# tpoisonooo/how-to-optimize-gemm

Measured on NVIDIA H100. Metric: SGEMM GFLOP/s (square N=4096 point of the 256..4096 sweep), higher is better.
Workload: dtype f16x2(scaled split-f32)

## Files before the change

how-to-optimize-gemm_b200/csrc/capi.cu:

```cuda
#include "../../include/b200gemm.h"

#include <cuda.h>
#include <cuda_runtime.h>
#include <stdio.h>
#include <stdlib.h>
#include <string.h>

#include <atomic>
#include <mutex>
#include <vector>

#include "gemm_ffma.cuh"
#include "gemm_generic.cuh"
#include "gemm_mxf4.cuh"
#include "gemm_tc.cuh"

using namespace b200;

namespace {

std::atomic<unsigned long long> g_launches{0};
int g_split_tail = 1;

struct KernelTimer {
// ... 58 lines not shown
  unsigned flag_slot = 0;
  struct FlagUser {
    cudaStream_t st = nullptr;
    cudaEvent_t ev = nullptr;
    bool used = false;
  } flag_user[kFlagSlots];
  std::mutex ws_mu;
  Scratch ws;
  cudaEvent_t ws_event = nullptr;
  cudaStream_t ws_stream = nullptr;
  bool ws_busy = false;
  struct MaxBuf {
    unsigned slot = 0;
    float* buf = nullptr;
    size_t cap = 0;
    int dirty[2] = {0, 0};
  } cmax, amax;
  cudaStream_t aux = nullptr;
  cudaEvent_t aux_fork = nullptr, aux_join = nullptr;
  std::mutex host_mu;
  Scratch scr[4];
  HostPipe pipe;
  std::vector<const void*> attr_done;
};
constexpr int kMaxDevices = 64;
DevCtx g_ctx[kMaxDevices];
std::mutex g_mu;

typedef CUresult (*EncodeTiledFn)(CUtensorMap*, CUtensorMapDataType, cuuint32_t, void*,
                                  const cuuint64_t*, const cuuint64_t*, const cuuint32_t*,
                                  const cuuint32_t*, CUtensorMapInterleave, CUtensorMapSwizzle,
                                  CUtensorMapL2promotion, CUtensorMapFloatOOBfill);
EncodeTiledFn g_encode = nullptr;

thread_local DevCtx* t_ctx = nullptr;
thread_local int t_bound_dev = -1;

int ensure_device() {
  int dev = -1;
  if (cudaGetDevice(&dev) != cudaSuccess || dev < 0 || dev >= kMaxDevices) { cudaGetLastError(); t_ctx = nullptr; return B200_ERR_NO_DEVICE; }
  if (t_bound_dev != dev) {
    if (cudaSetDevice(dev) != cudaSuccess) { cudaGetLastError(); t_ctx = nullptr; return B200_ERR_NO_DEVICE; }
    t_bound_dev = dev;
  }
  DevCtx* c = &g_ctx[dev];
  t_ctx = c;
// ... 25 lines not shown
  }
  for (auto& u : c->flag_user)
    if (!u.ev && cudaEventCreateWithFlags(&u.ev, cudaEventDisableTiming) != cudaSuccess) {
      cudaGetLastError(); u.ev = nullptr; c->ok = -1; return B200_ERR_NO_DEVICE;
    }
  c->dev = dev;
  c->sms = prop.multiProcessorCount;
  c->ok = 1;
  return 0;
}

template <typename Kern>
int ensure_smem_attr(Kern kern, int bytes) {
  const void* key = reinterpret_cast<const void*>(kern);
  {
    std::lock_guard<std::mutex> lk(g_mu);
    for (const void* k : t_ctx->attr_done) if (k == key) return 0;
  }
  cudaError_t e = cudaFuncSetAttribute(kern, cudaFuncAttributeMaxDynamicSharedMemorySize, bytes);
  if (e != cudaSuccess) { cudaGetLastError(); return (int)e; }
  std::lock_guard<std::mutex> lk(g_mu);
  t_ctx->attr_done.push_back(key);
  return 0;
}

struct MapKey {
  const void* ptr; int dtype; unsigned long long d0, d1, ld_bytes; unsigned b0, b1; int swz; int dev;
  unsigned long long d2, d2_bytes;
  bool operator==(const MapKey& o) const {
    return ptr == o.ptr && dtype == o.dtype && d0 == o.d0 && d1 == o.d1 && ld_bytes == o.ld_bytes &&
           b0 == o.b0 && b1 == o.b1 && swz == o.swz && dev == o.dev && d2 == o.d2 && d2_bytes == o.d2_bytes;
  }
};
struct MapEntry { MapKey key; CUtensorMap map; };
std::vector<MapEntry> g_maps;
size_t g_map_next = 0;
constexpr size_t kMapCache = 64;

int get_map(CUtensorMap* out, const void* ptr, CUtensorMapDataType dt, int elem_bytes,
            unsigned long long inner, unsigned long long rows, unsigned long long ld_bytes,
            unsigned box_inner, unsigned box_rows, int swizzle ,
            unsigned long long entries = 0, unsigned long long entry_bytes = 0) {
  MapKey key{ptr, (int)dt, inner, rows, ld_bytes, box_inner, box_rows, swizzle, t_ctx->dev, entries, entry_bytes};
  std::lock_guard<std::mutex> lk(g_mu);
  for (auto& e : g_maps)
    if (e.key == key) { *out = e.map; return 0; }
// ... 100 lines not shown
  if (cs == cudaStreamCaptureStatusNone) {
    if (u->used && (u->st != st || st == cudaStreamPerThread) && (e = cudaStreamWaitEvent(st, u->ev, 0)) != cudaSuccess) {
      cudaGetLastError();
      return (int)e;
    }
    *user = u;
  }
  if ((e = cudaMemsetAsync(*flags, 0, 1024 * sizeof(int), st)) != cudaSuccess) { cudaGetLastError(); return (int)e; }
  return 0;
}
void release_flag_slot(DevCtx::FlagUser* u, cudaStream_t st) {
  if (!u) return;
  if (cudaEventRecord(u->ev, st) != cudaSuccess) { cudaGetLastError(); return; }
  u->st = st;
  u->used = true;
}

int g_force_bn = 0;
int g_group_rows = 0;
constexpr int kStreamCDefault = 0;
int g_stream_c = -1;
int g_ffma_fat = -1;
int g_ffma_halves = 1;

struct Stack {
  int count;
  long long sa, sb, sc;
  const int32_t* offs;
};
long long grouped_tile_rows(int total_m, int groups) { return (total_m + 127LL) / 128 + groups; }

template <int KIND, int BN, int STAGES, typename OutT, class Prod = ProdSingle, int A_ROW_BYTES = 128, int AL = LAYOUT_K,
          int BL = KindTraits<KIND>::B_LAYOUT, bool EPI = false, int STACK = STACK_NONE, class ScaleT = TcScale>
int launch_tc(int m, int n, int k, const void* A, long long lda, int a_rows_total, int a_plane_rows,
              const void* B, long long ldb, int b_rows_total, int b_plane_rows, void* C, int ldc,
              const char* name, const Call& c, int chunk_k = 0, const float* row_max = nullptr,
              const float* col_max = nullptr, const Stack* stk = nullptr, const ScaleT* scl = nullptr) {
  using Cfg = TcConfig<KIND, BN, STAGES, Prod, A_ROW_BYTES, AL, BL>;
  using T = KindTraits<KIND>;
  constexpr bool FP8 = KIND == KIND_E4M3 || KIND == KIND_E4M3E5M2 || KIND == KIND_E5M2E4M3;
  constexpr bool BLK = std::is_same<ScaleT, TcBlockScale>::value || std::is_same<ScaleT, TcStackBlockScale>::value ||
                      std::is_same<ScaleT, TcBlockScaleQ8>::value;
  constexpr int smem = Cfg::SMEM_BYTES + (BLK ? STAGES * kBlkScaleStageBytes : 0);
  constexpr CUtensorMapDataType dt = KIND == KIND_F16 ? CU_TENSOR_MAP_DATA_TYPE_BFLOAT16
                                   : KIND == KIND_FP16 ? CU_TENSOR_MAP_DATA_TYPE_FLOAT16
                                   : KIND == KIND_TF32 ? CU_TENSOR_MAP_DATA_TYPE_FLOAT32
                                                       : CU_TENSOR_MAP_DATA_TYPE_UINT8;
  CUtensorMap tmA, tmB;
  constexpr int kswz = A_ROW_BYTES == 128 ? 1 : 3;
  unsigned long long ea = 0, eab = 0, eb = 0, ebb = 0;
  if constexpr (STACK != STACK_NONE) {
    const unsigned long long abytes = (unsigned long long)lda * T::ELEM, bbytes = (unsigned long long)ldb * T::ELEM;
    ea = stk->sa ? stk->count : 1; eab = stk->sa ? (unsigned long long)stk->sa * T::ELEM : a_rows_total * abytes;
    eb = stk->sb ? stk->count : 1; ebb = stk->sb ? (unsigned long long)stk->sb * T::ELEM : b_rows_total * bbytes;
  }
  int rc;
  if constexpr (Cfg::A_MN)
    rc = get_map(&tmA, A, dt, T::ELEM, m, a_rows_total, (unsigned long long)lda * T::ELEM, Cfg::MN_BOX_COLS, Cfg::BK, 1, ea,
                 eab);
  else
    rc = get_map(&tmA, A, dt, T::ELEM, k, a_rows_total, (unsigned long long)lda * T::ELEM, Cfg::BK, Cfg::BM, kswz, ea, eab);
  if (rc) return rc;
  if constexpr (!Cfg::B_MN)
// ... 5 lines not shown
  if (rc) return rc;
  TcParams p;
  p.C = C; p.ldc = ldc; p.M = m; p.N = n; p.K = k;
  p.tiles_m = STACK == STACK_GROUP ? (int)grouped_tile_rows(m, stk->count) : (m + Cfg::TILE_M - 1) / Cfg::TILE_M;
  p.tiles_n = (n + BN - 1) / BN;
  p.group_m = (g_group_rows > 0 ? g_group_rows : 2048) / Cfg::TILE_M;
  if (p.group_m < 1) p.group_m = 1;
  constexpr int OB = OutBytes<OutT>::V;
  p.vec_ok = aligned16(C) && ((long long)ldc * OB) % 16 == 0;
  if constexpr (STACK != STACK_NONE) p.vec_ok = p.vec_ok && stk->sc % (16 / OB) == 0;
  p.a_plane_rows = a_plane_rows; p.b_plane_rows = b_plane_rows;
  p.chunk_kb = chunk_k > 0 ? (chunk_k + Cfg::BK - 1) / Cfg::BK : (k + Cfg::BK - 1) / Cfg::BK;
  if (p.chunk_kb < 1) p.chunk_kb = 1;
  p.dbg_b_lbo = g_dbg_b_lbo; p.dbg_b_sbo = g_dbg_b_sbo;
  p.row_max = row_max; p.col_max = col_max;
  p.accumulate = c.acc;
  p.axpby = c.axpby; p.alpha = c.alpha; p.beta = c.beta;
  p.act = c.act;
  if constexpr (EPI) p.bias = c.bias;
  p.stream_c = g_stream_c < 0 ? (g_stream_c = (getenv("B200GEMM_STREAM_C") ? atoi(getenv("B200GEMM_STREAM_C")) : kStreamCDefault)) : g_stream_c;
  auto kern = [] {
    if constexpr (FP8) return gemm_tc_fp8_kernel<KIND, BN, STAGES, OutT, Prod, BLK, STACK>;
    else if constexpr (STACK != STACK_NONE) return gemm_tc_stacked_kernel<KIND, BN, STAGES, OutT, AL, BL, STACK>;
    else return gemm_tc_kernel<KIND, BN, STAGES, OutT, Prod, A_ROW_BYTES, AL, BL, EPI>;
  }();
  if (int arc = ensure_smem_attr(kern, smem)) return arc;
  TcStack ts{1, 0, 0, 0, nullptr};
  if constexpr (STACK != STACK_NONE) ts = TcStack{stk->count, stk->sa ? 1 : 0, stk->sb ? 1 : 0, stk->sc, stk->offs};
  [[maybe_unused]] ScaleT fp8_scale{};
  if constexpr (FP8) {
    fp8_scale = *scl;
    if constexpr (STACK != STACK_NONE) fp8_scale.st = ts;
  }
  int tiles = p.tiles_m * p.tiles_n * (STACK == STACK_GROUP ? 1 : ts.count);
  const int units_max = t_ctx->sms - c.sm_reserve > 2 ? t_ctx->sms - c.sm_reserve : t_ctx->sms;
  const int num_kb = (k + Cfg::BK - 1) / Cfg::BK;
  const int rem = tiles % units_max;
  int split = 1;
  if (!EPI && !FP8 && STACK != STACK_GROUP && STACK != STACK_KGROUP && g_split_tail && OB == 4 && rem > 0) {
    split = units_max / rem;
    if (split > 4) split = 4;
    if (split > num_kb / 8) split = num_kb / 8;
    if (split < 1) split = 1;
    if (rem * Cfg::EPI_WARPS > 1024) split = 1;
  }
  p.split = split;
  p.full_tiles = split > 1 ? tiles - rem : tiles;
  p.flags = t_ctx->flags;
  std::unique_lock<std::mutex> flag_lk;
  DevCtx::FlagUser* flag_user = nullptr;
  if (split > 1) {
    flag_lk = std::unique_lock<std::mutex>(t_ctx->flag_mu);
    if (int rc = take_flag_slot(c.st, &p.flags, &flag_user)) return rc;
  }
  const int items = p.full_tiles + (tiles - p.full_tiles) * split;
  const int units = items < units_max ? items : units_max;
  t_last_schedule = Schedule{tiles, split, p.full_tiles, units};
  g_ktimer.begin(c.st);
  {
    cudaError_t e;
    if constexpr (FP8) e = launch_pdl(kern, dim3(units), dim3(Cfg::THREADS), smem, c.st, 1, tmA, tmB, p, fp8_scale);
    else if constexpr (STACK != STACK_NONE) e = launch_pdl(kern, dim3(units), dim3(Cfg::THREADS), smem, c.st, 1, tmA, tmB, p, ts);
    else e = launch_pdl(kern, dim3(units), dim3(Cfg::THREADS), smem, c.st, 1, tmA, tmB, p);
    release_flag_slot(flag_user, c.st);
    if (e != cudaSuccess) { cudaGetLastError(); return (int)e; }
  }
  g_ktimer.end(c.st);
  g_launches++;
  t_last_kernel = name;
  return last_launch_status();
}

int pick_bn(int m, int n, bool allow256, bool allow192 = true, int batch = 1) {
  if (g_force_bn == 128 || (g_force_bn == 192 && allow192) || (g_force_bn == 256 && allow256)) return g_force_bn;
  const int cands[3] = {256, 192, 128};
  const double eff[3] = {1.00, 0.97, 0.80};
  int best = 128;
  double best_cost = 1e300;
  const int tm = (m + 127) / 128;
  for (int i = 0; i < 3; i++) {
    if (cands[i] == 256 && !allow256) continue;
    if (cands[i] == 192 && !allow192) continue;
    const long long tiles = (long long)tm * ((n + cands[i] - 1) / cands[i]) * batch;
    const long long waves = (tiles + t_ctx->sms - 1) / t_ctx->sms;
    const double cost = (double)waves * (cands[i] / eff[i] + 8.0);
    if (cost < best_cost) { best_cost = cost; best = cands[i]; }
// ... 214 lines not shown
  if (gy < 1) gy = 1;
  launch_pdl(split_planes_kernel<NP>, dim3(gx, gy, jobs), dim3(256), 0, st, 1, ja, jb);
  g_launches += 1;
  return last_launch_status();
}

struct PlaneGeom {
  int rows, cols, plane_rows;
  long long pitch;
  size_t bytes(int np) const { return (size_t)np * plane_rows * pitch * 2; }
};
inline PlaneGeom plane_geom(bool k_along_rows, int rows, int cols) {
  return PlaneGeom{rows, cols, k_along_rows ? b_plane_rows(rows) : rows, plane_pitch(cols)};
}
inline PlaneGeom geom_a(int op_a, int m, int k) { return op_a ? plane_geom(true, k, m) : plane_geom(false, m, k); }
inline PlaneGeom geom_b(int op_b, int k, int n) { return op_b ? plane_geom(false, n, k) : plane_geom(true, k, n); }

size_t split_ws_bytes(int np, int op_a, int op_b, int m, int n, int k, bool prepB = false) {
  const size_t a = round1024(geom_a(op_a, m, k).bytes(np));
  return prepB ? a : a + geom_b(op_b, k, n).bytes(np);
}

KernelNames kNamesBf16x3 = TC_NAMES("tc_bf16x3"), kNamesBf16x2 = TC_NAMES("tc_bf16x2"), kNamesF16x2 = TC_NAMES("tc_f16x2");

template <int NP>
int gemm_f32_split(int op_a, int op_b, int m, int n, int k, const float* A, int lda, const float* B, int ldb, float* C,
                   int ldc, const uint16_t* prepB, const Call& c) {
  const PlaneGeom ga = geom_a(op_a, m, k), gb = geom_b(op_b, k, n);
  WsLease ws(split_ws_bytes(NP, op_a, op_b, m, n, k, prepB != nullptr), c.st);
  if (ws.rc) return ws.rc;
  uint16_t* pA = reinterpret_cast<uint16_t*>(ws.base());
  const uint16_t* pB = prepB ? prepB : reinterpret_cast<uint16_t*>(ws.base() + round1024(ga.bytes(NP)));
  const SplitJob ja{A, lda, ga.rows, ga.cols, pA, ga.pitch, ga.plane_rows},
                 jb{B, ldb, gb.rows, gb.cols, const_cast<uint16_t*>(pB), gb.pitch, gb.plane_rows};
  if (int rc = launch_split<NP>(ja, jb, prepB ? 1 : 2, c.st)) return rc;
  using Prod = typename std::conditional<NP == 3, ProdX3, ProdX2>::type;
  return with_layout(op_a, op_b, [&](auto L) {
    using Lay = decltype(L);
    return launch_tc<KIND_F16, 128, NP == 3 ? 4 : 6, float, Prod, 64, Lay::AL, Lay::BL>(
        m, n, k, pA, ga.pitch, NP * ga.plane_rows, ga.plane_rows, pB, gb.pitch, NP * gb.plane_rows, gb.plane_rows, C, ldc,
        (NP == 3 ? kNamesBf16x3 : kNamesBf16x2)[Lay::idx][2], c, g_split_chunk_k[NP == 3 ? 0 : 1]);
  });
}

struct F16Operand {
  const uint16_t* planes;
  long long pitch;
  int plane_rows;
  const float* maxv;
};

int launch_f16_split_rows(const float* A, long long lda, int rows, int cols, float* rmax, uint16_t* planes,
                          long long pitch, int plane_rows, cudaStream_t st) {
  int blocks = (plane_rows + 7) / 8;
  const int cap = t_ctx->sms * 16;
  if (blocks > cap) blocks = cap;
  if (blocks < 1) blocks = 1;
  if (cols <= 1024) launch_pdl(split_f16_rows_kernel<4>, dim3(blocks), dim3(256), 0, st, 1, A, (long long)lda, rows, cols, rmax, planes, pitch, plane_rows);
  else if (cols <= 2048) launch_pdl(split_f16_rows_kernel<8>, dim3(blocks), dim3(256), 0, st, 1, A, (long long)lda, rows, cols, rmax, planes, pitch, plane_rows);
  else if (cols <= 4096) launch_pdl(split_f16_rows_kernel<16>, dim3(blocks), dim3(256), 0, st, 1, A, (long long)lda, rows, cols, rmax, planes, pitch, plane_rows);
  else launch_pdl(split_f16_rows_kernel<0>, dim3(blocks), dim3(256), 0, st, 1, A, (long long)lda, rows, cols, rmax, planes, pitch, plane_rows);
  g_launches++;
  return last_launch_status();
}

int launch_f16_split_cols(const float* B, long long ldb, int rows, int cols, float* cmax, uint16_t* planes,
                          long long pitch, int plane_rows, float* zero_buf, int zero_n, cudaStream_t st) {
  launch_pdl(col_absmax_kernel, dim3((cols + 1023) / 1024, (rows + 15) / 16), dim3(256), 0, st, 1, B, (long long)ldb, rows, cols,
             reinterpret_cast<unsigned int*>(cmax));
  const int gx = (int)((pitch + 2047) / 2048);
  int gy = (t_ctx->sms * 8 + gx - 1) / gx;
  if (gy > (plane_rows + 1) / 2) gy = (plane_rows + 1) / 2;
  if (gy < 1) gy = 1;
  if (zero_buf && zero_n > gx * 2048) {
    cudaMemsetAsync(zero_buf, 0, (size_t)zero_n * 4, st);
    zero_buf = nullptr;
  }
  launch_pdl(split_f16_cols_kernel, dim3(gx, gy), dim3(256), 0, st, 1, B, (long long)ldb, rows, cols, (const float*)cmax, planes, pitch, plane_rows, zero_buf, zero_n);
  g_launches += 2;
  return last_launch_status();
}

int gemm_f16x2_core(int op_a, int op_b, int m, int n, int k, const F16Operand& a, const F16Operand& b, float* C, int ldc,
                    const Call& c) {
  constexpr int NP = 2;
  return with_layout(op_a, op_b, [&](auto L) {
    using Lay = decltype(L);
    return launch_tc<KIND_FP16, 128, 6, float, ProdX2, 64, Lay::AL, Lay::BL>(
        m, n, k, a.planes, a.pitch, NP * a.plane_rows, a.plane_rows, b.planes, b.pitch, NP * b.plane_rows, b.plane_rows, C,
        ldc, kNamesF16x2[Lay::idx][2], c, g_split_chunk_k[2], a.maxv, b.maxv);
  });
}

int cmax_reserve(DevCtx::MaxBuf& mb, int n, float** cur, float** other, int* other_dirty) {
  if (mb.cap < (size_t)n) {
    size_t cap = mb.cap ? 2 * mb.cap : 16384;
    if (cap < (size_t)n) cap = (size_t)n;
    if (mb.buf) { cudaDeviceSynchronize(); cudaFree(mb.buf); }
    mb.buf = nullptr; mb.cap = 0;
    cudaError_t e = cudaMalloc(&mb.buf, 2 * cap * sizeof(float));
    if (e == cudaSuccess) e = cudaMemset(mb.buf, 0, 2 * cap * sizeof(float));
    if (e != cudaSuccess) { cudaGetLastError(); return (int)e; }
    mb.cap = cap;
    mb.dirty[0] = mb.dirty[1] = 0;
  }
  const unsigned slot = mb.slot++ & 1u;
  *cur = mb.buf + slot * mb.cap;
  *other = mb.buf + (slot ^ 1u) * mb.cap;
  *other_dirty = mb.dirty[slot ^ 1u];
  mb.dirty[slot ^ 1u] = 0;
  mb.dirty[slot] = n;
  return 0;
}
// ... 889 lines not shown

const char* b200_gemm_strerror(int code) {
  switch (code) {
    case B200_OK: return "ok";
    case B200_ERR_BAD_ARG: return "bad argument";
    case B200_ERR_NO_DEVICE: return "no usable sm_90 CUDA device (there is no CPU fallback)";
    case B200_ERR_UNSUPPORTED: return "mode not supported for these operands";
    case B200_ERR_TENSORMAP: return "cuTensorMapEncodeTiled failed";
    case B200_ERR_NCCL: return "NCCL failure (b200_nccl_last_error has the text)";
    default: return code > 0 ? cudaGetErrorString((cudaError_t)code) : "unknown";
  }
}

const char* b200_gemm_last_kernel(void) { return t_last_kernel; }
unsigned long long b200_gemm_launch_count(void) { return g_launches.load(); }
int b200_gemm_default_f32_mode(void) { return resolve_f32_mode(B200_F32_AUTO); }
void b200_gemm_set_default_f32_mode(int mode) {
  if (mode >= 0 && mode != B200_F32_AUTO && mode <= B200_F32_F16X2) g_default_f32_mode.store(mode);
}
void b200_gemm_debug_set_b_desc(int lbo_bytes, int sbo_bytes) { g_dbg_b_lbo = lbo_bytes; g_dbg_b_sbo = sbo_bytes; }
void b200_gemm_debug_set_bn(int bn) { g_force_bn = bn; }
void b200_gemm_debug_set_pdl(int v) { g_pdl = (v & 1) != 0; g_prepass_fork = (v & 2) == 0; }
void b200_gemm_debug_set_dynamic_sched(int) {}
void b200_gemm_debug_set_cta_group(int) {}
void b200_gemm_debug_set_split_tail(int on) { g_split_tail = on; }
void b200_gemm_debug_last_schedule(int* tiles, int* split, int* full_tiles, int* ctas) {
  const Schedule& s = t_last_schedule;
  if (tiles) *tiles = s.tiles;
  if (split) *split = s.split;
  if (full_tiles) *full_tiles = s.full_tiles;
  if (ctas) *ctas = s.ctas;
}
void b200_gemm_debug_set_epilogue(int) {}
void b200_gemm_debug_set_group_rows(int rows) { g_group_rows = rows; }
void b200_gemm_debug_set_ffma_variant(int v) { g_ffma_halves = v & 1; g_ffma_fat = v < 0 ? -1 : (v >> 1) & 1; }
void b200_gemm_debug_set_split_chunk(int x3_k, int x2_k) {
  g_split_chunk_k[0] = x3_k < 0 ? kSplitChunkDefault[0] : x3_k;
  g_split_chunk_k[1] = x2_k < 0 ? kSplitChunkDefault[1] : x2_k;
  g_split_chunk_k[2] = x2_k < 0 ? kSplitChunkDefault[2] : x2_k;
}
void b200_gemm_debug_kernel_timing(int enable) { g_ktimer.on = enable != 0; g_ktimer.n = 0; }
int b200_gemm_debug_kernel_time_ms(double* sum_ms) {
  double sum = 0;
  int cnt = 0;
  for (int i = 0; i < g_ktimer.n; i++) {
    float ms = 0.f;
    if (cudaEventSynchronize(g_ktimer.ev[i][1]) == cudaSuccess &&
// ... 520 lines not shown
```

how-to-optimize-gemm_b200/csrc/gemm_tc.cuh:

```cuda
#pragma once
#include <cuda_fp16.h>
#include <string.h>
#include <type_traits>

#include "ptx.cuh"
#include "wgmma.cuh"

namespace b200 {

enum Layout { LAYOUT_K = 0, LAYOUT_MN = 1 };

template <int KIND> struct KindTraits;
template <> struct KindTraits<KIND_F16>  { static constexpr int ELEM = 2; static constexpr int B_LAYOUT = LAYOUT_MN; };
template <> struct KindTraits<KIND_FP16> { static constexpr int ELEM = 2; static constexpr int B_LAYOUT = LAYOUT_MN; };
template <> struct KindTraits<KIND_TF32> { static constexpr int ELEM = 4; static constexpr int B_LAYOUT = LAYOUT_K; };
template <> struct KindTraits<KIND_I8>   { static constexpr int ELEM = 1; static constexpr int B_LAYOUT = LAYOUT_K; };
template <> struct KindTraits<KIND_E4M3> { static constexpr int ELEM = 1; static constexpr int B_LAYOUT = LAYOUT_K; };
template <> struct KindTraits<KIND_E4M3E5M2> { static constexpr int ELEM = 1; static constexpr int B_LAYOUT = LAYOUT_K; };
template <> struct KindTraits<KIND_E5M2E4M3> { static constexpr int ELEM = 1; static constexpr int B_LAYOUT = LAYOUT_K; };

struct ProdSingle {
  static constexpr int N = 1, NPA = 1, NPB = 1;
  __host__ __device__ static constexpr int ia(int) { return 0; }
  __host__ __device__ static constexpr int ib(int) { return 0; }
// ... 68 lines not shown
  static constexpr int B_BOX_BYTES = B_MN ? MN_BOX_BYTES : BN * A_ROW_BYTES;
  static constexpr int B_PLANE = B_BOXES * B_BOX_BYTES;
  static constexpr int A_STAGE = Prod::NPA * A_PLANE;
  static constexpr int B_STAGE = Prod::NPB * B_PLANE;
  static constexpr int STAGE_BYTES = A_STAGE + B_STAGE;
  using MMA = Wgmma<KIND, BN, A_MN ? 1 : 0, B_MN ? 1 : 0>;
  static constexpr int MMA_K = MMA::K;
  static constexpr int MMAS_PER_STAGE = BK / MMA_K;
  static constexpr int A_KADV = A_MN ? MMA_K * 128 : MMA_K * T::ELEM;
  static constexpr int B_KADV = B_MN ? MMA_K * 128 : MMA_K * T::ELEM;
  static constexpr int ACC = BN / 2;
  static constexpr int SMEM_BYTES = 1024  + STAGES * STAGE_BYTES + 2 * STAGES * 8;
  static constexpr int THREADS = 128 * (1 + CONSUMERS);
  static_assert(SMEM_BYTES <= 232448, "exceeds the 227 KB dynamic shared memory of sm_90");
  static_assert(!REGACC || BN <= 128, "register accumulation keeps two 64 x BN fp32 tiles per consumer in registers");
  static_assert(T::ELEM == 2 || (!A_MN && !B_MN && Prod::NPA == 1 && Prod::NPB == 1 && A_ROW_BYTES == 128),
                "tf32 / int8: K-major A and B, single plane, 128-byte rows");
  static_assert(!B_MN || BN % MN_BOX_COLS == 0, "MN-major B is staged in 128-byte column blocks");
  static_assert(!A_MN || (A_BOXES == CONSUMERS && A_BOXES * MN_BOX_BYTES == A_PLANE),
                "MN-major A: one 64-column box per consumer warpgroup, the bytes of a K-major A plane");
  static_assert(B_PLANE == BN * A_ROW_BYTES, "a B plane holds BN x BK elements in either layout");
};

__device__ __forceinline__ void tile_coords(int t, int tiles_m, int tiles_n, int group_m, int& mb,
                                            int& nb) {
  const int per_group = group_m * tiles_n;
  const int g = t / per_group;
  const int first_m = g * group_m;
  const int rows = min(group_m, tiles_m - first_m);
  const int r = t - g * per_group;
  mb = first_m + r % rows;
  nb = r / rows;
}

__host__ __device__ __forceinline__ int pow2_exp(float maxv) {
  uint32_t bits;
#ifdef __CUDA_ARCH__
  bits = __float_as_uint(maxv);
#else
  memcpy(&bits, &maxv, 4);
#endif
  const int ef = (int)((bits >> 23) & 0xFF);
  const uint32_t mant = bits & 0x7FFFFFu;
#ifdef __CUDA_ARCH__
  const int sub = (31 - __clz(mant | 1u)) - 148;
#else
  const int sub = (31 - __builtin_clz(mant | 1u)) - 148;
#endif
// ... 134 lines not shown
  const uint16_t* bias = reinterpret_cast<const uint16_t*>(p.bias);
  const bool bias_vec = (reinterpret_cast<uintptr_t>(bias) & 3) == 0;
  const int ce[2] = {0, 0};
#pragma unroll
  for (int j = 0; j < BN / 8; j++) {
    const int col = col0 + 8 * j;
    float b[2] = {-0.f, -0.f};
    if (bias != nullptr && col < p.N) {
      uint32_t h;
      if (bias_vec && col + 1 < p.N) h = __ldg(reinterpret_cast<const unsigned int*>(bias + col));
      else h = (uint32_t)__ldg(reinterpret_cast<const unsigned short*>(bias + col)) |
               (col + 1 < p.N ? (uint32_t)__ldg(reinterpret_cast<const unsigned short*>(bias + col + 1)) << 16 : 0u);
      b[0] = c16_to_f32<Bias16>(h & 0xFFFFu);
      b[1] = c16_to_f32<Bias16>(h >> 16);
    }
#pragma unroll
    for (int h = 0; h < 2; h++)
      store_pair<OutT, float, ACT>(p, row0 + 8 * h, col, acc[4 * j + 2 * h], acc[4 * j + 2 * h + 1], fold, false, al, be,
                                   0, ce, 0.f, 0.f, b[0], b[1]);
  }
}

template <int KIND, int BN, int STAGES, typename OutT, class Prod, int A_ROW_BYTES, int AL = LAYOUT_K,
          int BL = KindTraits<KIND>::B_LAYOUT, bool EPI = false>
__global__ void __launch_bounds__((TcConfig<KIND, BN, STAGES, Prod, A_ROW_BYTES, AL, BL>::THREADS), 1)
gemm_tc_kernel(const __grid_constant__ CUtensorMap tmA, const __grid_constant__ CUtensorMap tmB,
               const TcParams p) {
  using Cfg = TcConfig<KIND, BN, STAGES, Prod, A_ROW_BYTES, AL, BL>;
  using MMA = typename Cfg::MMA;
  using Acc = typename MMA::Acc;
  static_assert(!EPI || (KindTraits<KIND>::ELEM == 2 && !Cfg::REGACC &&
                         (std::is_same<OutT, float>::value || OutBytes<OutT>::V == 2)),
                "bias / activation epilogue: 16-bit single-plane kinds with fp32 or 16-bit C");

  extern __shared__ uint8_t smem_raw[];
  const uint32_t smem_base = (smem_u32(smem_raw) + 1023u) & ~1023u;
  const uint32_t sA = smem_base;
  const uint32_t sB = sA + STAGES * Cfg::A_STAGE;
  const uint32_t bar_full = sB + STAGES * Cfg::B_STAGE;
  const uint32_t bar_empty = bar_full + 8 * STAGES;

  const int warp = threadIdx.x >> 5;
  const int lane = threadIdx.x & 31;
  if (threadIdx.x == 0) {
    tma_prefetch_desc(&tmA);
    tma_prefetch_desc(&tmB);
    for (int i = 0; i < STAGES; i++) {
      mbar_init(bar_full + 8 * i, 1);
      mbar_init(bar_empty + 8 * i, Cfg::CONSUMERS);
    }
    fence_barrier_init();
  }
  __syncthreads();
  griddep_launch();
  griddep_wait();

  const int num_tiles = p.tiles_m * p.tiles_n;
  const int num_items = p.full_tiles + (num_tiles - p.full_tiles) * p.split;
  const int num_kb = (p.K + Cfg::BK - 1) / Cfg::BK;

  if (warp < 4) {
    setmaxnreg_dec<40>();
    if (warp == 0 && lane == 0) {
      int s = 0;
      uint32_t ph = 0;
      for (int w = blockIdx.x; w < num_items; w += gridDim.x) {
        const WorkItem it = work_item(w, p, num_kb);
        int mb, nb;
        tile_coords(it.tile, p.tiles_m, p.tiles_n, p.group_m, mb, nb);
        const int m0 = mb * Cfg::BM, n0 = nb * BN;
        for (int kb = it.kb0; kb < it.kb1; kb++) {
          mbar_wait(bar_empty + 8 * s, ph ^ 1);
          const uint32_t full = bar_full + 8 * s;
          mbar_arrive_expect_tx(full, Cfg::STAGE_BYTES);
          if constexpr (Cfg::A_MN) {
#pragma unroll
            for (int pa = 0; pa < Prod::NPA; pa++)
#pragma unroll
              for (int j = 0; j < Cfg::A_BOXES; j++)
                tma_load_2d(sA + s * Cfg::A_STAGE + pa * Cfg::A_PLANE + j * Cfg::MN_BOX_BYTES, &tmA, full,
                            m0 + j * Cfg::MN_BOX_COLS, pa * p.a_plane_rows + kb * Cfg::BK);
          } else {
#pragma unroll
            for (int pa = 0; pa < Prod::NPA; pa++)
              tma_load_2d(sA + s * Cfg::A_STAGE + pa * Cfg::A_PLANE, &tmA, full, kb * Cfg::BK, pa * p.a_plane_rows + m0);
          }
          if constexpr (!Cfg::B_MN) {
            if constexpr (Prod::NPB == 1) {
              tma_load_2d(sB + s * Cfg::B_STAGE, &tmB, full, kb * Cfg::BK, n0);
            } else {
#pragma unroll
              for (int pb = 0; pb < Prod::NPB; pb++)
                tma_load_2d(sB + s * Cfg::B_STAGE + pb * Cfg::B_PLANE, &tmB, full, kb * Cfg::BK, pb * p.b_plane_rows + n0);
            }
          } else {
#pragma unroll
            for (int pb = 0; pb < Prod::NPB; pb++)
#pragma unroll
              for (int j = 0; j < Cfg::B_BOXES; j++)
                tma_load_2d(sB + s * Cfg::B_STAGE + pb * Cfg::B_PLANE + j * Cfg::B_BOX_BYTES, &tmB, full,
                            n0 + j * Cfg::B_BOX_COLS, pb * p.b_plane_rows + kb * Cfg::BK);
          }
          if (++s == STAGES) { s = 0; ph ^= 1; }
        }
      }
    }
  } else {
    setmaxnreg_inc<232>();
    const int cw = warp / 4 - 1;
    const int ew = warp - 4;
    const bool wg_leader = (threadIdx.x & 127) == 0;
    const uint32_t b_lbo = p.dbg_b_lbo ? (uint32_t)p.dbg_b_lbo : (uint32_t)Cfg::B_BOX_BYTES;
    const uint32_t b_sbo = p.dbg_b_sbo ? (uint32_t)p.dbg_b_sbo : 1024u;
    int s = 0;
    uint32_t ph = 0;
    Acc acc[Cfg::ACC];
    float sum[Cfg::REGACC ? Cfg::ACC : 1];
    for (int w = blockIdx.x; w < num_items; w += gridDim.x) {
      const WorkItem it = work_item(w, p, num_kb);
      int mb, nb;
      tile_coords(it.tile, p.tiles_m, p.tiles_n, p.group_m, mb, nb);
      const int m0 = mb * Cfg::BM, n0 = nb * BN;
      const int chunk = Cfg::REGACC ? p.chunk_kb : it.kb1 - it.kb0;
      for (int c0 = it.kb0; c0 < it.kb1; c0 += chunk) {
        const int c1 = min(c0 + chunk, it.kb1);
        int prev = -1;
        for (int kb = c0; kb < c1; kb++) {
          mbar_wait(bar_full + 8 * s, ph);
          const uint32_t a0 = sA + s * Cfg::A_STAGE + cw * Cfg::A_WG;
          const uint32_t b0 = sB + s * Cfg::B_STAGE;
          wgmma_fence();
#pragma unroll
          for (int pr = 0; pr < Prod::N; pr++) {
#pragma unroll
            for (int k = 0; k < Cfg::MMAS_PER_STAGE; k++) {
              uint64_t ad, bd;
              if constexpr (Cfg::A_MN)
                ad = make_sdesc(a0 + Prod::ia(pr) * Cfg::A_PLANE + k * Cfg::A_KADV, Cfg::MN_BOX_BYTES, 1024, SWZ_128B);
              else
                ad = make_sdesc(a0 + Prod::ia(pr) * Cfg::A_PLANE + k * Cfg::A_KADV, 16, Cfg::A_SBO, Cfg::A_SWZ);
              if constexpr (Cfg::B_MN)
                bd = make_sdesc(b0 + Prod::ib(pr) * Cfg::B_PLANE + k * Cfg::B_KADV, b_lbo, b_sbo, SWZ_128B);
              else if constexpr (Prod::NPB == 1)
                bd = make_sdesc(b0 + k * Cfg::B_KADV, 16, Cfg::A_SBO, Cfg::A_SWZ);
              else
                bd = make_sdesc(b0 + Prod::ib(pr) * Cfg::B_PLANE + k * Cfg::B_KADV, 16, Cfg::A_SBO, Cfg::A_SWZ);
              MMA::mma(acc, ad, bd, ((kb - c0) | k | pr) != 0 ? 1u : 0u);
            }
          }
          wgmma_commit();
          wgmma_wait<1>();
          if (prev >= 0 && wg_leader) mbar_arrive(bar_empty + 8 * prev);
          prev = s;
          if (++s == STAGES) { s = 0; ph ^= 1; }
        }
        wgmma_wait<0>();
        wgmma_fence_regs(acc);
        if (prev >= 0 && wg_leader) mbar_arrive(bar_empty + 8 * prev);
        if constexpr (Cfg::REGACC) {
#pragma unroll
          for (int i = 0; i < Cfg::ACC; i++) sum[i] = c0 == it.kb0 ? acc[i] : __fadd_rn(sum[i], acc[i]);
        }
      }

      int* flag = p.flags + (it.tile - p.full_tiles) * Cfg::EPI_WARPS + ew;
      if (it.part > 0) {
        if (lane == 0) {
          const long long t0 = clock64();
          while (true) {
            int v;
            asm volatile("ld.acquire.gpu.global.s32 %0, [%1];" : "=r"(v) : "l"(flag) : "memory");
            if (v == it.part) break;
            if (clock64() - t0 > 4000000000LL) { asm volatile("trap;"); }
          }
        }
        __syncwarp();
      }
      const bool fold = p.accumulate != 0 || it.part > 0 || (p.axpby && p.beta != 0.f);
      const float al = p.axpby ? p.alpha : 1.f;
      const float be = (p.axpby && it.part == 0) ? p.beta : 1.f;
      const int row0 = m0 + ew * 16 + (lane >> 2);
      const int col0 = n0 + 2 * (lane & 3);
      int re[2] = {0, 0};
      float sc[2] = {0.f, 0.f}, bi[2] = {0.f, 0.f};
#pragma unroll
      for (int h = 0; h < 2; h++) {
        const int row = row0 + 8 * h;
        if (row < p.M) {
// ... 23 lines not shown
              if (col + e < p.N) ce[e] = pow2_exp(__ldg(p.col_max + col + e));
          }
#pragma unroll
          for (int h = 0; h < 2; h++) {
            if constexpr (Cfg::REGACC)
              store_pair<OutT>(p, row0 + 8 * h, col, sum[4 * j + 2 * h], sum[4 * j + 2 * h + 1], fold, it.part > 0, al, be,
                               re[h], ce, sc[h], bi[h]);
            else
              store_pair<OutT>(p, row0 + 8 * h, col, acc[4 * j + 2 * h], acc[4 * j + 2 * h + 1], fold, it.part > 0, al,
                               be, re[h], ce, sc[h], bi[h]);
          }
        }
      }
      if (w >= p.full_tiles && p.split > 1) {
        __threadfence();
        __syncwarp();
        if (lane == 0) {
          const int nv = it.part + 1 == p.split ? 0 : it.part + 1;
          asm volatile("st.release.gpu.global.s32 [%0], %1;" ::"l"(flag), "r"(nv) : "memory");
        }
      }
    }
  }
}

struct StackEntry {
  int tile0, tiles_m;
  int a_row, a_entry;
  int b_entry;
  int M;
  long long c_off;
  int k0, k_len;
  int entry;
};
template <int STACK>
__device__ __forceinline__ StackEntry stack_entry(int tile, const TcParams& p, const TcStack& st, const int* grp_end,
                                                  const int* grp_tile) {
  StackEntry se;
  int e;
  if constexpr (STACK == STACK_GROUP) {
    e = group_of(grp_tile, st.count, tile / p.tiles_n);
    se.tile0 = grp_tile[e] * p.tiles_n;
    se.tiles_m = grp_tile[e + 1] - grp_tile[e];
    se.a_row = grp_end[e];
    se.M = grp_end[e + 1] - grp_end[e];
    se.c_off = (long long)grp_end[e] * p.ldc;
// ... 1068 lines not shown
```

how-to-optimize-gemm_b200/csrc/ptx.cuh:

```cuda
#pragma once
#include <cuda.h>
#include <cuda_runtime.h>
#include <math.h>
#include <stdint.h>

namespace b200 {

__device__ __forceinline__ uint32_t smem_u32(const void* p) {
  return static_cast<uint32_t>(__cvta_generic_to_shared(p));
}

__device__ __forceinline__ void mbar_init(uint32_t bar, uint32_t count) {
  asm volatile("mbarrier.init.shared::cta.b64 [%0], %1;" ::"r"(bar), "r"(count) : "memory");
}
__device__ __forceinline__ void fence_barrier_init() {
  asm volatile("fence.mbarrier_init.release.cluster;" ::: "memory");
}
__device__ __forceinline__ void fence_proxy_async() {
  asm volatile("fence.proxy.async.shared::cta;" ::: "memory");
}
__device__ __forceinline__ void mbar_arrive_expect_tx(uint32_t bar, uint32_t bytes) {
  asm volatile("mbarrier.arrive.expect_tx.shared::cta.b64 _, [%0], %1;" ::"r"(bar), "r"(bytes)
               : "memory");
}
__device__ __forceinline__ void mbar_arrive(uint32_t bar) {
  asm volatile("mbarrier.arrive.shared::cta.b64 _, [%0];" ::"r"(bar) : "memory");
}
__device__ __forceinline__ bool mbar_try_wait(uint32_t bar, uint32_t parity) {
  uint32_t ok;
  asm volatile(
      "{\n\t.reg .pred p;\n\t"
      "mbarrier.try_wait.parity.shared::cta.b64 p, [%1], %2;\n\t"
      "selp.u32 %0, 1, 0, p;\n\t}"
      : "=r"(ok)
      : "r"(bar), "r"(parity)
      : "memory");
  return ok != 0;
}
__device__ __forceinline__ void mbar_wait(uint32_t bar, uint32_t parity) {
  if (mbar_try_wait(bar, parity)) return;
  const long long t0 = clock64();
  while (!mbar_try_wait(bar, parity)) {
    if (clock64() - t0 > 4000000000LL) { asm volatile("trap;"); }
  }
}

__device__ __forceinline__ void tma_prefetch_desc(const CUtensorMap* m) {
  asm volatile("prefetch.tensormap [%0];" ::"l"(reinterpret_cast<uint64_t>(m)) : "memory");
}
__device__ __forceinline__ void tma_load_2d(uint32_t dst_smem, const CUtensorMap* m, uint32_t bar,
                                            int c0, int c1) {
  asm volatile(
      "cp.async.bulk.tensor.2d.shared::cluster.global.tile.mbarrier::complete_tx::bytes "
      "[%0], [%1, {%3, %4}], [%2];"
      ::"r"(dst_smem), "l"(reinterpret_cast<uint64_t>(m)), "r"(bar), "r"(c0), "r"(c1)
      : "memory");
}
__device__ __forceinline__ void tma_load_3d(uint32_t dst_smem, const CUtensorMap* m, uint32_t bar,
                                            int c0, int c1, int c2) {
  asm volatile(
      "cp.async.bulk.tensor.3d.shared::cluster.global.tile.mbarrier::complete_tx::bytes "
      "[%0], [%1, {%3, %4, %5}], [%2];"
      ::"r"(dst_smem), "l"(reinterpret_cast<uint64_t>(m)), "r"(bar), "r"(c0), "r"(c1), "r"(c2)
      : "memory");
}
__device__ __forceinline__ void tma_load_2d_hint(uint32_t dst_smem, const CUtensorMap* m,
                                                 uint32_t bar, int c0, int c1, uint64_t policy) {
  asm volatile(
      "cp.async.bulk.tensor.2d.shared::cluster.global.tile.mbarrier::complete_tx::bytes"
      ".L2::cache_hint [%0], [%1, {%3, %4}], [%2], %5;"
      ::"r"(dst_smem), "l"(reinterpret_cast<uint64_t>(m)), "r"(bar), "r"(c0), "r"(c1), "l"(policy)
      : "memory");
}

enum MmaKind { KIND_F16 = 0 , KIND_TF32 = 1, KIND_I8 = 2, KIND_FP16 = 3 ,
               KIND_E4M3 = 4 , KIND_E4M3E5M2 = 5 , KIND_E5M2E4M3 = 6  };
enum Swz { SWZ_128B = 1, SWZ_64B = 2 };

__device__ __forceinline__ uint64_t make_sdesc(uint32_t smem_addr, uint32_t lbo_bytes, uint32_t sbo_bytes, uint32_t swz) {
  uint64_t d = 0;
  d |= (uint64_t)((smem_addr & 0x3FFFF) >> 4);
  d |= (uint64_t)((lbo_bytes >> 4) & 0x3FFF) << 16;
  d |= (uint64_t)((sbo_bytes >> 4) & 0x3FFF) << 32;
  d |= (uint64_t)swz << 62;
  return d;
}
// ... 89 lines not shown
```

Baseline: 187,500.

## Pair CTAs in 2-wide clusters with TMA multicast of B planes for split-f32 GEMM

Adds a cluster-of-two launch mode, enabled by default, for the bf16x2 and f16x2 split-f32 WGMMA kernels. The two CTAs in a pair take adjacent M tiles with the same N tile. Each CTA loads one of the two B planes and multicasts it to both CTAs' shared memory, which halves per-CTA B traffic from global memory and L2. Empty barriers now count consumers from both CTAs, with cross-CTA mbarrier arrivals and cluster syncs at start and end. The costs are tighter cross-CTA coupling of the pipeline stages, a possible idle CTA when tiles_m is odd, and cluster occupancy limits on how many units can run.

Result: faster. 189,800 (median of 6 runs) (+1.2%).

```diff
diff --git a/how-to-optimize-gemm_b200/csrc/capi.cu b/how-to-optimize-gemm_b200/csrc/capi.cu
--- a/how-to-optimize-gemm_b200/csrc/capi.cu
+++ b/how-to-optimize-gemm_b200/csrc/capi.cu
@@ -104,6 +104,7 @@
   Scratch scr[4];
   HostPipe pipe;
   std::vector<const void*> attr_done;
+  std::vector<std::pair<const void*, int>> max_clusters;
 };
 constexpr int kMaxDevices = 64;
 DevCtx g_ctx[kMaxDevices];
@@ -175,6 +176,26 @@
   std::lock_guard<std::mutex> lk(g_mu);
   t_ctx->attr_done.push_back(key);
   return 0;
+}
+
+template <typename Kern>
+int max_pair_clusters(Kern kern, int smem, int threads) {
+  const void* key = reinterpret_cast<const void*>(kern);
+  {
+    std::lock_guard<std::mutex> lk(g_mu);
+    for (const auto& e : t_ctx->max_clusters) if (e.first == key) return e.second;
+  }
+  cudaLaunchConfig_t cfg = {};
+  cfg.gridDim = dim3(2 * t_ctx->sms); cfg.blockDim = dim3(threads); cfg.dynamicSmemBytes = smem;
+  cudaLaunchAttribute at;
+  at.id = cudaLaunchAttributeClusterDimension;
+  at.val.clusterDim.x = 2; at.val.clusterDim.y = 1; at.val.clusterDim.z = 1;
+  cfg.attrs = &at; cfg.numAttrs = 1;
+  int n = 0;
+  if (cudaOccupancyMaxActiveClusters(&n, kern, &cfg) != cudaSuccess) { cudaGetLastError(); return 0; }
+  std::lock_guard<std::mutex> lk(g_mu);
+  t_ctx->max_clusters.push_back({key, n});
+  return n;
 }
 
 struct MapKey {
@@ -321,6 +342,8 @@
 int g_stream_c = -1;
 int g_ffma_fat = -1;
 int g_ffma_halves = 1;
+constexpr int kCtaGroupDefault = 2;
+int g_cta_group = kCtaGroupDefault;
 
 struct Stack {
   int count;
@@ -330,7 +353,7 @@
 long long grouped_tile_rows(int total_m, int groups) { return (total_m + 127LL) / 128 + groups; }
 
 template <int KIND, int BN, int STAGES, typename OutT, class Prod = ProdSingle, int A_ROW_BYTES = 128, int AL = LAYOUT_K,
-          int BL = KindTraits<KIND>::B_LAYOUT, bool EPI = false, int STACK = STACK_NONE, class ScaleT = TcScale>
+          int BL = KindTraits<KIND>::B_LAYOUT, bool EPI = false, int STACK = STACK_NONE, class ScaleT = TcScale, int CM = 1>
 int launch_tc(int m, int n, int k, const void* A, long long lda, int a_rows_total, int a_plane_rows,
               const void* B, long long ldb, int b_rows_total, int b_plane_rows, void* C, int ldc,
               const char* name, const Call& c, int chunk_k = 0, const float* row_max = nullptr,
@@ -338,6 +361,7 @@
   using Cfg = TcConfig<KIND, BN, STAGES, Prod, A_ROW_BYTES, AL, BL>;
   using T = KindTraits<KIND>;
   constexpr bool FP8 = KIND == KIND_E4M3 || KIND == KIND_E4M3E5M2 || KIND == KIND_E5M2E4M3;
+  static_assert(CM == 1 || (!FP8 && STACK == STACK_NONE && !EPI), "CTA pairs: the single-matrix split-mode kernel only");
   constexpr bool BLK = std::is_same<ScaleT, TcBlockScale>::value || std::is_same<ScaleT, TcStackBlockScale>::value ||
                       std::is_same<ScaleT, TcBlockScaleQ8>::value;
   constexpr int smem = Cfg::SMEM_BYTES + (BLK ? STAGES * kBlkScaleStageBytes : 0);
@@ -389,7 +413,7 @@
   auto kern = [] {
     if constexpr (FP8) return gemm_tc_fp8_kernel<KIND, BN, STAGES, OutT, Prod, BLK, STACK>;
     else if constexpr (STACK != STACK_NONE) return gemm_tc_stacked_kernel<KIND, BN, STAGES, OutT, AL, BL, STACK>;
-    else return gemm_tc_kernel<KIND, BN, STAGES, OutT, Prod, A_ROW_BYTES, AL, BL, EPI>;
+    else return gemm_tc_kernel<KIND, BN, STAGES, OutT, Prod, A_ROW_BYTES, AL, BL, EPI, CM>;
   }();
   if (int arc = ensure_smem_attr(kern, smem)) return arc;
   TcStack ts{1, 0, 0, 0, nullptr};
@@ -400,7 +424,15 @@
     if constexpr (STACK != STACK_NONE) fp8_scale.st = ts;
   }
   int tiles = p.tiles_m * p.tiles_n * (STACK == STACK_GROUP ? 1 : ts.count);
-  const int units_max = t_ctx->sms - c.sm_reserve > 2 ? t_ctx->sms - c.sm_reserve : t_ctx->sms;
+  int units_max = t_ctx->sms - c.sm_reserve > 2 ? t_ctx->sms - c.sm_reserve : t_ctx->sms;
+  const int out_tiles = tiles;
+  if constexpr (CM == 2) {
+    tiles = (p.tiles_m + 1) / 2 * p.tiles_n;
+    const int clusters = max_pair_clusters(kern, smem, Cfg::THREADS);
+    if (clusters < 1) return B200_ERR_NO_DEVICE;
+    units_max = clusters < units_max / 2 ? clusters : units_max / 2;
+    if (units_max < 1) units_max = 1;
+  }
   const int num_kb = (k + Cfg::BK - 1) / Cfg::BK;
   const int rem = tiles % units_max;
   int split = 1;
@@ -409,7 +441,7 @@
     if (split > 4) split = 4;
     if (split > num_kb / 8) split = num_kb / 8;
     if (split < 1) split = 1;
-    if (rem * Cfg::EPI_WARPS > 1024) split = 1;
+    if (rem * CM * Cfg::EPI_WARPS > 1024) split = 1;
   }
   p.split = split;
   p.full_tiles = split > 1 ? tiles - rem : tiles;
@@ -422,13 +454,22 @@
   }
   const int items = p.full_tiles + (tiles - p.full_tiles) * split;
   const int units = items < units_max ? items : units_max;
-  t_last_schedule = Schedule{tiles, split, p.full_tiles, units};
+  int full_out = p.full_tiles;
+  if constexpr (CM == 2) {
+    full_out = out_tiles;
+    for (int u = p.full_tiles; u < tiles; u++) {
+      int ub, nb;
+      tile_coords(u, (p.tiles_m + 1) / 2, p.tiles_n, p.group_m / 2 > 1 ? p.group_m / 2 : 1, ub, nb);
+      full_out -= 2 * ub + 1 < p.tiles_m ? 2 : 1;
+    }
+  }
+  t_last_schedule = Schedule{out_tiles, split, full_out, units * CM};
   g_ktimer.begin(c.st);
   {
     cudaError_t e;
     if constexpr (FP8) e = launch_pdl(kern, dim3(units), dim3(Cfg::THREADS), smem, c.st, 1, tmA, tmB, p, fp8_scale);
     else if constexpr (STACK != STACK_NONE) e = launch_pdl(kern, dim3(units), dim3(Cfg::THREADS), smem, c.st, 1, tmA, tmB, p, ts);
-    else e = launch_pdl(kern, dim3(units), dim3(Cfg::THREADS), smem, c.st, 1, tmA, tmB, p);
+    else e = launch_pdl(kern, dim3(units * CM), dim3(Cfg::THREADS), smem, c.st, CM, tmA, tmB, p);
     release_flag_slot(flag_user, c.st);
     if (e != cudaSuccess) { cudaGetLastError(); return (int)e; }
   }
@@ -689,6 +730,11 @@
 }
 
 KernelNames kNamesBf16x3 = TC_NAMES("tc_bf16x3"), kNamesBf16x2 = TC_NAMES("tc_bf16x2"), kNamesF16x2 = TC_NAMES("tc_f16x2");
+template <class F>
+int with_cta_group(int m, F&& f) {
+  if (g_cta_group == 2 && m > 128) return f(std::integral_constant<int, 2>());
+  return f(std::integral_constant<int, 1>());
+}
 
 template <int NP>
 int gemm_f32_split(int op_a, int op_b, int m, int n, int k, const float* A, int lda, const float* B, int ldb, float* C,
@@ -704,9 +750,18 @@
   using Prod = typename std::conditional<NP == 3, ProdX3, ProdX2>::type;
   return with_layout(op_a, op_b, [&](auto L) {
     using Lay = decltype(L);
-    return launch_tc<KIND_F16, 128, NP == 3 ? 4 : 6, float, Prod, 64, Lay::AL, Lay::BL>(
-        m, n, k, pA, ga.pitch, NP * ga.plane_rows, ga.plane_rows, pB, gb.pitch, NP * gb.plane_rows, gb.plane_rows, C, ldc,
-        (NP == 3 ? kNamesBf16x3 : kNamesBf16x2)[Lay::idx][2], c, g_split_chunk_k[NP == 3 ? 0 : 1]);
+    if constexpr (NP == 3) {
+      return launch_tc<KIND_F16, 128, 4, float, Prod, 64, Lay::AL, Lay::BL>(
+          m, n, k, pA, ga.pitch, NP * ga.plane_rows, ga.plane_rows, pB, gb.pitch, NP * gb.plane_rows, gb.plane_rows, C, ldc,
+          kNamesBf16x3[Lay::idx][2], c, g_split_chunk_k[0]);
+    } else {
+      return with_cta_group(m, [&](auto G) {
+        constexpr int CM = decltype(G)::value;
+        return launch_tc<KIND_F16, 128, 6, float, Prod, 64, Lay::AL, Lay::BL, false, STACK_NONE, TcScale, CM>(
+            m, n, k, pA, ga.pitch, NP * ga.plane_rows, ga.plane_rows, pB, gb.pitch, NP * gb.plane_rows, gb.plane_rows, C,
+            ldc, kNamesBf16x2[Lay::idx][2], c, g_split_chunk_k[1]);
+      });
+    }
   });
 }
 
@@ -753,9 +808,12 @@
   constexpr int NP = 2;
   return with_layout(op_a, op_b, [&](auto L) {
     using Lay = decltype(L);
-    return launch_tc<KIND_FP16, 128, 6, float, ProdX2, 64, Lay::AL, Lay::BL>(
-        m, n, k, a.planes, a.pitch, NP * a.plane_rows, a.plane_rows, b.planes, b.pitch, NP * b.plane_rows, b.plane_rows, C,
-        ldc, kNamesF16x2[Lay::idx][2], c, g_split_chunk_k[2], a.maxv, b.maxv);
+    return with_cta_group(m, [&](auto G) {
+      constexpr int CM = decltype(G)::value;
+      return launch_tc<KIND_FP16, 128, 6, float, ProdX2, 64, Lay::AL, Lay::BL, false, STACK_NONE, TcScale, CM>(
+          m, n, k, a.planes, a.pitch, NP * a.plane_rows, a.plane_rows, b.planes, b.pitch, NP * b.plane_rows, b.plane_rows,
+          C, ldc, kNamesF16x2[Lay::idx][2], c, g_split_chunk_k[2], a.maxv, b.maxv);
+    });
   });
 }
 
@@ -1691,7 +1749,7 @@
 void b200_gemm_debug_set_bn(int bn) { g_force_bn = bn; }
 void b200_gemm_debug_set_pdl(int v) { g_pdl = (v & 1) != 0; g_prepass_fork = (v & 2) == 0; }
 void b200_gemm_debug_set_dynamic_sched(int) {}
-void b200_gemm_debug_set_cta_group(int) {}
+void b200_gemm_debug_set_cta_group(int cg) { g_cta_group = cg == 1 || cg == 2 ? cg : kCtaGroupDefault; }
 void b200_gemm_debug_set_split_tail(int on) { g_split_tail = on; }
 void b200_gemm_debug_last_schedule(int* tiles, int* split, int* full_tiles, int* ctas) {
   const Schedule& s = t_last_schedule;
diff --git a/how-to-optimize-gemm_b200/csrc/gemm_tc.cuh b/how-to-optimize-gemm_b200/csrc/gemm_tc.cuh
--- a/how-to-optimize-gemm_b200/csrc/gemm_tc.cuh
+++ b/how-to-optimize-gemm_b200/csrc/gemm_tc.cuh
@@ -114,8 +114,8 @@
   static_assert(B_PLANE == BN * A_ROW_BYTES, "a B plane holds BN x BK elements in either layout");
 };
 
-__device__ __forceinline__ void tile_coords(int t, int tiles_m, int tiles_n, int group_m, int& mb,
-                                            int& nb) {
+__host__ __device__ __forceinline__ void tile_coords(int t, int tiles_m, int tiles_n, int group_m, int& mb,
+                                                     int& nb) {
   const int per_group = group_m * tiles_n;
   const int g = t / per_group;
   const int first_m = g * group_m;
@@ -296,7 +296,7 @@
 }
 
 template <int KIND, int BN, int STAGES, typename OutT, class Prod, int A_ROW_BYTES, int AL = LAYOUT_K,
-          int BL = KindTraits<KIND>::B_LAYOUT, bool EPI = false>
+          int BL = KindTraits<KIND>::B_LAYOUT, bool EPI = false, int CM = 1>
 __global__ void __launch_bounds__((TcConfig<KIND, BN, STAGES, Prod, A_ROW_BYTES, AL, BL>::THREADS), 1)
 gemm_tc_kernel(const __grid_constant__ CUtensorMap tmA, const __grid_constant__ CUtensorMap tmB,
                const TcParams p) {
@@ -306,6 +306,7 @@
   static_assert(!EPI || (KindTraits<KIND>::ELEM == 2 && !Cfg::REGACC &&
                          (std::is_same<OutT, float>::value || OutBytes<OutT>::V == 2)),
                 "bias / activation epilogue: 16-bit single-plane kinds with fp32 or 16-bit C");
+  static_assert(CM == 1 || (CM == 2 && Prod::NPB == 2 && !EPI), "CTA pairs: one B plane per CTA of the pair");
 
   extern __shared__ uint8_t smem_raw[];
   const uint32_t smem_base = (smem_u32(smem_raw) + 1023u) & ~1023u;
@@ -321,15 +322,19 @@
     tma_prefetch_desc(&tmB);
     for (int i = 0; i < STAGES; i++) {
       mbar_init(bar_full + 8 * i, 1);
-      mbar_init(bar_empty + 8 * i, Cfg::CONSUMERS);
+      mbar_init(bar_empty + 8 * i, CM * Cfg::CONSUMERS);
     }
     fence_barrier_init();
   }
-  __syncthreads();
+  if constexpr (CM == 2) cluster_sync();
+  else __syncthreads();
   griddep_launch();
   griddep_wait();
 
-  const int num_tiles = p.tiles_m * p.tiles_n;
+  const int rank = (int)(blockIdx.x % CM);
+  const int units_m = (p.tiles_m + CM - 1) / CM;
+  const int group_u = CM == 1 ? p.group_m : max(p.group_m / CM, 1);
+  const int num_tiles = units_m * p.tiles_n;
   const int num_items = p.full_tiles + (num_tiles - p.full_tiles) * p.split;
   const int num_kb = (p.K + Cfg::BK - 1) / Cfg::BK;
 
@@ -338,11 +343,11 @@
     if (warp == 0 && lane == 0) {
       int s = 0;
       uint32_t ph = 0;
-      for (int w = blockIdx.x; w < num_items; w += gridDim.x) {
+      for (int w = blockIdx.x / CM; w < num_items; w += gridDim.x / CM) {
         const WorkItem it = work_item(w, p, num_kb);
         int mb, nb;
-        tile_coords(it.tile, p.tiles_m, p.tiles_n, p.group_m, mb, nb);
-        const int m0 = mb * Cfg::BM, n0 = nb * BN;
+        tile_coords(it.tile, units_m, p.tiles_n, group_u, mb, nb);
+        const int m0 = (mb * CM + rank) * Cfg::BM, n0 = nb * BN;
         for (int kb = it.kb0; kb < it.kb1; kb++) {
           mbar_wait(bar_empty + 8 * s, ph ^ 1);
           const uint32_t full = bar_full + 8 * s;
@@ -359,7 +364,17 @@
             for (int pa = 0; pa < Prod::NPA; pa++)
               tma_load_2d(sA + s * Cfg::A_STAGE + pa * Cfg::A_PLANE, &tmA, full, kb * Cfg::BK, pa * p.a_plane_rows + m0);
           }
-          if constexpr (!Cfg::B_MN) {
+          if constexpr (CM == 2) {
+            if constexpr (!Cfg::B_MN) {
+              tma_load_2d_mc(sB + s * Cfg::B_STAGE + rank * Cfg::B_PLANE, &tmB, full, kb * Cfg::BK,
+                             rank * p.b_plane_rows + n0, 0x3);
+            } else {
+#pragma unroll
+              for (int j = 0; j < Cfg::B_BOXES; j++)
+                tma_load_2d_mc(sB + s * Cfg::B_STAGE + rank * Cfg::B_PLANE + j * Cfg::B_BOX_BYTES, &tmB, full,
+                               n0 + j * Cfg::B_BOX_COLS, rank * p.b_plane_rows + kb * Cfg::BK, 0x3);
+            }
+          } else if constexpr (!Cfg::B_MN) {
             if constexpr (Prod::NPB == 1) {
               tma_load_2d(sB + s * Cfg::B_STAGE, &tmB, full, kb * Cfg::BK, n0);
             } else {
@@ -390,10 +405,18 @@
     uint32_t ph = 0;
     Acc acc[Cfg::ACC];
     float sum[Cfg::REGACC ? Cfg::ACC : 1];
-    for (int w = blockIdx.x; w < num_items; w += gridDim.x) {
+    auto release = [&](int st) {
+      if constexpr (CM == 1) mbar_arrive(bar_empty + 8 * st);
+      else {
+        mbar_arrive(bar_empty + 8 * st);
+        mbar_arrive_cluster(bar_empty + 8 * st, rank ^ 1);
+      }
+    };
+    for (int w = blockIdx.x / CM; w < num_items; w += gridDim.x / CM) {
       const WorkItem it = work_item(w, p, num_kb);
       int mb, nb;
-      tile_coords(it.tile, p.tiles_m, p.tiles_n, p.group_m, mb, nb);
+      tile_coords(it.tile, units_m, p.tiles_n, group_u, mb, nb);
+      mb = mb * CM + rank;
       const int m0 = mb * Cfg::BM, n0 = nb * BN;
       const int chunk = Cfg::REGACC ? p.chunk_kb : it.kb1 - it.kb0;
       for (int c0 = it.kb0; c0 < it.kb1; c0 += chunk) {
@@ -424,20 +447,21 @@
           }
           wgmma_commit();
           wgmma_wait<1>();
-          if (prev >= 0 && wg_leader) mbar_arrive(bar_empty + 8 * prev);
+          if (prev >= 0 && wg_leader) release(prev);
           prev = s;
           if (++s == STAGES) { s = 0; ph ^= 1; }
         }
         wgmma_wait<0>();
         wgmma_fence_regs(acc);
-        if (prev >= 0 && wg_leader) mbar_arrive(bar_empty + 8 * prev);
+        if (prev >= 0 && wg_leader) release(prev);
         if constexpr (Cfg::REGACC) {
 #pragma unroll
           for (int i = 0; i < Cfg::ACC; i++) sum[i] = c0 == it.kb0 ? acc[i] : __fadd_rn(sum[i], acc[i]);
         }
       }
 
-      int* flag = p.flags + (it.tile - p.full_tiles) * Cfg::EPI_WARPS + ew;
+      if (CM == 2 && mb >= p.tiles_m) continue;
+      int* flag = p.flags + ((it.tile - p.full_tiles) * CM + rank) * Cfg::EPI_WARPS + ew;
       if (it.part > 0) {
         if (lane == 0) {
           const long long t0 = clock64();
@@ -507,6 +531,7 @@
       }
     }
   }
+  if constexpr (CM == 2) cluster_sync();
 }
 
 struct StackEntry {
diff --git a/how-to-optimize-gemm_b200/csrc/ptx.cuh b/how-to-optimize-gemm_b200/csrc/ptx.cuh
--- a/how-to-optimize-gemm_b200/csrc/ptx.cuh
+++ b/how-to-optimize-gemm_b200/csrc/ptx.cuh
@@ -25,6 +25,14 @@
 }
 __device__ __forceinline__ void mbar_arrive(uint32_t bar) {
   asm volatile("mbarrier.arrive.shared::cta.b64 _, [%0];" ::"r"(bar) : "memory");
+}
+__device__ __forceinline__ void mbar_arrive_cluster(uint32_t bar, uint32_t cta) {
+  uint32_t remote;
+  asm volatile("mapa.shared::cluster.u32 %0, %1, %2;" : "=r"(remote) : "r"(bar), "r"(cta));
+  asm volatile("mbarrier.arrive.shared::cluster.b64 _, [%0];" ::"r"(remote) : "memory");
+}
+__device__ __forceinline__ void cluster_sync() {
+  asm volatile("barrier.cluster.arrive.release.aligned;\n\tbarrier.cluster.wait.acquire.aligned;" ::: "memory");
 }
 __device__ __forceinline__ bool mbar_try_wait(uint32_t bar, uint32_t parity) {
   uint32_t ok;
@@ -62,6 +70,14 @@
       "cp.async.bulk.tensor.3d.shared::cluster.global.tile.mbarrier::complete_tx::bytes "
       "[%0], [%1, {%3, %4, %5}], [%2];"
       ::"r"(dst_smem), "l"(reinterpret_cast<uint64_t>(m)), "r"(bar), "r"(c0), "r"(c1), "r"(c2)
+      : "memory");
+}
+__device__ __forceinline__ void tma_load_2d_mc(uint32_t dst_smem, const CUtensorMap* m, uint32_t bar, int c0, int c1,
+                                               uint16_t cta_mask) {
+  asm volatile(
+      "cp.async.bulk.tensor.2d.shared::cluster.global.tile.mbarrier::complete_tx::bytes.multicast::cluster "
+      "[%0], [%1, {%3, %4}], [%2], %5;"
+      ::"r"(dst_smem), "l"(reinterpret_cast<uint64_t>(m)), "r"(bar), "r"(c0), "r"(c1), "h"(cta_mask)
       : "memory");
 }
 __device__ __forceinline__ void tma_load_2d_hint(uint32_t dst_smem, const CUtensorMap* m,
```
